# hinike/cairo

Measured on AMD Instinct MI355X. Metric: encoded Mpixels/s (p-frame, q=16) at 1/2/4/8 MI355X; bit-exact vs ref, higher is better.
Workload: dtype int16

## Files before the change

### cairo_amd/__init__.py

```python
from __future__ import annotations

import ctypes
import os
from dataclasses import dataclass

import numpy as np

_HERE = os.path.dirname(os.path.abspath(__file__))
LIB_PATH = os.path.join(_HERE, "_lib", "libcairo_amd.so")

BLOCK_DESC = np.dtype(
    [
        ("block_type", "<u4"),
        ("prediction_target", "u1"),
        ("pad", "u1"),
        ("motion_x", "<i2"),
        ("motion_y", "<i2"),
        ("sp_pred", "u1"),
        ("sp_amount", "u1"),
        ("sp_index", "u1"),
        ("q_index", "u1"),
        ("variance", "<i2"),
    ]
)
# ... 362 lines not shown
    feed: np.ndarray | None = None
    feed_bits: int = 0
    feed_status: int = 0


def _view(addr: int, dtype, count: int) -> np.ndarray:
    buf = (ctypes.c_char * (count * np.dtype(dtype).itemsize)).from_address(addr)
    return np.frombuffer(buf, dtype=dtype, count=count)


class Context:

    def __init__(self, width: int, height: int, ring: int = 4, device: int = 0, stages: int = 96):
        self.L = lib()
        self.width, self.height, self.ring, self.device = width, height, ring, device
        self.wa, self.ha = (width + 15) & ~15, (height + 15) & ~15
        self.wmb, self.hmb = self.wa // 16, self.ha // 16
        p = ctypes.c_void_p()
        _ck(self.L.cairo_ctx_create_ex(width, height, ring, device, stages, ctypes.byref(p)), "cairo_ctx_create")
        self.h = p
        self._keep = {}

    def close(self) -> None:
        if self.h:
            self.L.cairo_ctx_destroy(self.h)
            self.h = None

    def __del__(self):
        try:
            self.close()
        except Exception:
            pass

    @property
    def stages(self) -> int:
        return int(self.L.cairo_ctx_stages(self.h))

    def submit(self, rgb, index: int, inter: bool, quality: int, on_device: bool = False,
               fmt: int = FMT_RGB24, pitch: int = 0, src_size=None, crop=None) -> int:
        t = ctypes.c_int()
        if src_size is not None or crop is not None:
            if src_size is None:
                raise ValueError("crop needs src_size")
            s = _source(src_size, crop)
            ptr = _scaled_source_ptr(rgb, on_device, fmt, src_size, pitch)
            _ck(self.L.cairo_ctx_submit_scaled(self.h, ptr, fmt, pitch, ctypes.byref(s), index, int(inter), quality,
                                               ctypes.byref(t)), "cairo_ctx_submit_scaled")
            return t.value
        ptr = rgb if on_device else _host_frame_fmt(rgb, fmt, self.width, self.height, pitch)
        if fmt == FMT_RGB24 and not pitch:
            _ck(
                self.L.cairo_ctx_submit(self.h, ptr, int(on_device), index, int(inter), quality, ctypes.byref(t)),
                "cairo_ctx_submit",
            )
        else:
            _ck(self.L.cairo_ctx_submit_fmt(self.h, ptr, int(on_device), fmt, pitch, index, int(inter), quality,
                                            ctypes.byref(t)), "cairo_ctx_submit_fmt")
        if not on_device:
            self._keep[t.value] = rgb
        return t.value

    def wait(self, ticket: int, copy: bool = True) -> FrameOutputs:
        r = _FrameResult()
        st = self.L.cairo_ctx_wait(self.h, ticket, ctypes.byref(r))
        if st != EVX_SUCCESS:
            raise CairoError("cairo_ctx_wait", st, self.timeout_info() if st == EVX_ERROR_HARDWAREFAIL else None)
        self._keep.pop(ticket, None)
        return self._outputs(r, copy)

    ACCT_FIELDS = ("coder_tasks", "coder_total", "coder_group_wait", "coder_window", "coder_search", "coder_inter",
                   "coder_dequeue", "coder_mbs", "helper_tasks", "helper_total", "helper_wait", "helper_deblock",
                   "helper_search", "helper_catchup", "helper_dequeue", "helper_chunks",
                   "win_bytes", "win_spec_unused_bytes", "zero_mv_bytes", "gran_poll_bytes", "rec_poll_bytes",
                   "win_stages", "searched_tasks", "inter_tasks", "coder_xform", "coder_publish", "coder_drain",
                   "coder_vm0", "coder_records", "coder_prebarrier", "coder_store_tail",
                   "search_eval", "search_barrier", "search_select", "subpel_eval", "subpel_barrier",
                   "subpel_select", "db_inputs", "db_filter", "db_write",
                   "search_passes", "search_mbs_2pass", "search_mbs_3pass", "search_mbs_4pass",
                   "coder_xform_copy", "coder_copy_mbs", "coder_xform_coded", "coder_coded_mbs",
                   "helper_carry", "carry_bytes",
                   "coder_prologue_fresh", "coder_prologue_records", "helper_group_start",
                   "start_older_searched", "start_ref1_searched", "start_older_idle", "start_ref1_idle",
                   "older_searched", "older_idle", "ref1_idle",
                   "flag_set", "fallback_polls", "fallback_full", "lvl2_runs", "idle_groups", "idle_group_time")

    def read_acct(self, reset: bool = False) -> dict:
        w = np.zeros(len(self.ACCT_FIELDS), np.uint64)
        _ck(self.L.cairo_ctx_read_acct(self.h, _ptr(w), len(w), int(reset)), "cairo_ctx_read_acct")
        return {k: int(w[i]) for i, k in enumerate(self.ACCT_FIELDS)}

    def timeout_info(self) -> dict | None:
        w = np.zeros(16, np.int32)
        _ck(self.L.cairo_ctx_timeout_info(self.h, _ptr(w), 16), "cairo_ctx_timeout_info")
        if not w[0]:
            return None
        d = {k: int(w[i]) for i, k in enumerate(TIMEOUT_FIELDS)}
        d["kind"] = WAIT_KINDS.get(d["kind"], str(d["kind"]))
        d["seen"] = (d.pop("seen_hi") & 0xFFFFFFFF) << 32 | (d.pop("seen_lo") & 0xFFFFFFFF)
        return d

    def _outputs(self, r, copy: bool) -> FrameOutputs:
        ny, nc = r.wa * r.ha, (r.wa // 2) * (r.ha // 2)
        mbs = r.wmb * r.hmb
        has_coef = bool(r.coef_y)
        feed = _view(r.feed, np.uint32, (r.feed_bits + 31) // 32) if r.feed_status == FEED_VALID else None
        out = FrameOutputs(
            _view(r.block_table, BLOCK_DESC, mbs),
            _view(r.coef_y, np.int16, ny).reshape(r.ha, r.wa) if has_coef else None,
            _view(r.coef_u, np.int16, nc).reshape(r.ha // 2, r.wa // 2) if has_coef else None,
            _view(r.coef_v, np.int16, nc).reshape(r.ha // 2, r.wa // 2) if has_coef else None,
            feed, int(r.feed_bits), int(r.feed_status),
        )
        if copy:
            cp = lambda a: None if a is None else a.copy()
            out = FrameOutputs(cp(out.table), cp(out.coef_y), cp(out.coef_u), cp(out.coef_v), cp(out.feed),
                               out.feed_bits, out.feed_status)
        return out

    def set_outputs(self, outputs: int) -> None:
        _ck(self.L.cairo_ctx_set_outputs(self.h, outputs), "cairo_ctx_set_outputs")

    def fetch_coef(self, ticket: int):
        r = _FrameResult()
        _ck(self.L.cairo_ctx_fetch_coef(self.h, ticket, ctypes.byref(r)), "cairo_ctx_fetch_coef")
        ny, nc = self.wa * self.ha, (self.wa // 2) * (self.ha // 2)
        return (_view(r.coef_y, np.int16, ny).reshape(self.ha, self.wa).copy(),
                _view(r.coef_u, np.int16, nc).reshape(self.ha // 2, self.wa // 2).copy(),
                _view(r.coef_v, np.int16, nc).reshape(self.ha // 2, self.wa // 2).copy())

    def set_metrics(self, sse: bool = True, ssim: bool = True, keep_recon: bool = False, flags: int | None = None) -> None:
        if flags is None:
            flags = (METRIC_SSE if sse else 0) | (METRIC_SSIM if ssim else 0) | (KEEP_RECON if keep_recon else 0)
        _ck(self.L.cairo_ctx_set_metrics(self.h, flags), "cairo_ctx_set_metrics")

    def set_input_color(self, range: int, matrix: int) -> None:
        _ck(self.L.cairo_ctx_set_input_color(self.h, range, matrix), "cairo_ctx_set_input_color")

    def set_output_color(self, range: int, matrix: int) -> None:
        _ck(self.L.cairo_ctx_set_output_color(self.h, range, matrix), "cairo_ctx_set_output_color")

    def frame_metrics(self, ticket: int) -> dict:
        m = _FrameMetrics()
        _ck(self.L.cairo_ctx_frame_metrics(self.h, ticket, ctypes.byref(m)), "cairo_ctx_frame_metrics")
        return _metrics_dict(m)

    def fetch_recon_planes(self, ticket: int):
        y = np.empty((self.ha, self.wa), np.int16)
        u = np.empty((self.ha // 2, self.wa // 2), np.int16)
        v = np.empty_like(u)
        _ck(self.L.cairo_ctx_fetch_recon_planes(self.h, ticket, _ptr(y), _ptr(u), _ptr(v)),
            "cairo_ctx_fetch_recon_planes")
        return y, u, v

    def fetch_recon(self, ticket: int, fmt: int, pitch: int = 0, out: np.ndarray | None = None) -> np.ndarray:
        nb, _ = frame_layout(fmt, self.width, self.height, pitch)
        if out is None:
            out = np.zeros(nb, np.uint8)
        elif not isinstance(out, np.ndarray) or out.dtype != np.uint8 or out.nbytes != nb or \
                not out.flags["C_CONTIGUOUS"]:
            raise ValueError(f"out must be a C-contiguous uint8 array of {nb} bytes")
        _ck(self.L.cairo_ctx_fetch_recon(self.h, ticket, fmt, pitch, _ptr(out)), "cairo_ctx_fetch_recon")
        return out

    def release(self, ticket: int) -> None:
        _ck(self.L.cairo_ctx_release(self.h, ticket), "cairo_ctx_release")

    def encode_frame(self, rgb, index: int, inter: bool, quality: int, on_device: bool = False,
# ... 513 lines not shown
```

### cairo_amd/csrc/kernels.h

```cpp
#pragma once

#include <hip/hip_runtime.h>
#include <stddef.h>
#include <stdint.h>

#include "evx_defs.h"

namespace cairo {

struct PlaneSet {
  int16_t* y;
  int16_t* u;
  int16_t* v;
};

__host__ __device__ inline PlaneSet ring_slot(int16_t* base, size_t slot_elems, int wa, int ha,
                                              int k) {
  PlaneSet p;
  p.y = base + (size_t)k * slot_elems;
  p.u = p.y + (size_t)wa * ha;
  p.v = p.u + (size_t)(wa / 2) * (ha / 2);
  return p;
}

constexpr int kGranulesPerMB = 192;
constexpr int kGranuleStride = 193;

__host__ __device__ inline uint32_t pack_inter_desc(const BlockDesc& d) {
  return (d.block_type & 7u) | ((uint32_t)(d.prediction_target & 3) << 3) | ((uint32_t)(d.sp_pred & 1) << 5) |
         ((uint32_t)(d.sp_amount & 1) << 6) | ((uint32_t)(d.sp_index & 15) << 7) |
         (((uint32_t)d.motion_x & 0x7Fu) << 11) | (((uint32_t)d.motion_y & 0x7Fu) << 18);
}
__host__ __device__ inline BlockDesc unpack_inter_desc(uint32_t w) {
  BlockDesc d;
  d.block_type = w & 7u;
  d.prediction_target = (uint8_t)((w >> 3) & 3);
  d.pad = 0;
  d.sp_pred = (uint8_t)((w >> 5) & 1);
  d.sp_amount = (uint8_t)((w >> 6) & 1);
  d.sp_index = (uint8_t)((w >> 7) & 15);
  d.motion_x = (int16_t)((int32_t)(w << 14) >> 25);
  d.motion_y = (int16_t)((int32_t)(w << 7) >> 25);
  d.q_index = 0;
  d.variance = 0;
  return d;
}

constexpr int kStampPhases = 12;
constexpr int kDbStamps = 256;
constexpr int kIStamps = 12;
__host__ __device__ inline size_t stamp_frame_words(int wmb, int hmb) {
  return (size_t)wmb * hmb * kStampPhases + (size_t)hmb * kDbStamps;
}

struct TimeoutInfo {
  static constexpr int kKind = 0;
  static constexpr int kEpoch = 1;
  static constexpr int kIndex = 2;
  static constexpr int kRow = 3;
  static constexpr int kMember = 4;
  static constexpr int kNeed = 5;
  static constexpr int kOn = 6;
  static constexpr int kSeenLo = 7;
  static constexpr int kSeenHi = 8;
  static constexpr int kClaim = 9;
  static constexpr int kWords = 16;
};
enum TimeoutKind : int32_t {
  kWaitRecords = 1,
  kWaitGranule = 2,
  kWaitPrevProgress = 3,
  kWaitRowAbove = 4,
  kWaitBatch = 5,
  kWaitInjected = 6,
  kWaitHostMark = 9,
};

#ifndef CAIRO_ACCT
#define CAIRO_ACCT 0
#endif
constexpr int kAcctShards = 64, kAcctWords = 66;
struct Acct {
  static constexpr int kCoderTasks = 0, kCoderTotal = 1, kCoderGroupWait = 2, kCoderWindow = 3, kCoderSearch = 4,
                       kCoderInter = 5, kCoderDequeue = 6, kCoderMBs = 7;
  static constexpr int kHelperTasks = 8, kHelperTotal = 9, kHelperWait = 10, kHelperDeblock = 11, kHelperSearch = 12,
                       kHelperCatchup = 13, kHelperDequeue = 14, kHelperChunks = 15;
  static constexpr int kWinBytes = 16, kWinSpecUnused = 17, kZeroMvBytes = 18, kGranPollBytes = 19,
                       kRecPollBytes = 20, kWinStages = 21, kSearchedTasks = 22, kInterTasks = 23;
  static constexpr int kCoderXform = 24, kCoderPublish = 25, kCoderDrain = 26;
  static constexpr int kCoderVm0 = 27, kCoderRecords = 28, kCoderPreBarrier = 29;
  static constexpr int kCoderStoreTail = 30;
  static constexpr int kSrchEval = 31, kSrchBarrier = 32, kSrchSelect = 33, kSubEval = 34, kSubBarrier = 35,
                       kSubSelect = 36;
  static constexpr int kDbInputs = 37, kDbFilter = 38, kDbWrite = 39;
  static constexpr int kSrchPasses = 40, kSrchPasses2 = 41, kSrchPasses3 = 42, kSrchPasses4 = 43;
  static constexpr int kCoderXformCopy = 44, kCoderCopyMBs = 45, kCoderXformCoded = 46, kCoderCodedMBs = 47;
  static constexpr int kHelperCarry = 48, kCarryBytes = 49;
  static constexpr int kCoderProFresh = 50, kCoderProRecords = 51, kHelperGroupStart = 52;
  static constexpr int kStartOlderSearched = 53, kStartRef1Searched = 54, kStartOlderIdle = 55, kStartRef1Idle = 56,
                       kOlderSearched = 57, kOlderIdle = 58, kRef1Idle = 59;
  static constexpr int kFlagSet = 60, kFallbackPolls = 61, kFallbackFull = 62, kLvl2Runs = 63;
  static constexpr int kIdleGroups = 64, kIdleGroupTime = 65;
};

#ifndef CAIRO_MAX_BATCH
#define CAIRO_MAX_BATCH 48
#endif
constexpr int kMaxBatch = CAIRO_MAX_BATCH;
constexpr int kMaxGroup = 16;
constexpr int kMaxPush = kMaxRing;

struct FrameDesc {
  const uint8_t* rgb;
  const uint8_t* host_rgb;
  int index;
  int inter;
  int quality;
  uint32_t epoch;
  int slot;
  int decode;
  PlaneSet recon[kMaxRing];
  PlaneSet stale;
  PlaneSet coef;
  PlaneSet push[kMaxPush];
  int npush;
  PlaneSet coef_prev;
  uint64_t* progress;
  const uint64_t* prev_progress;
  const uint64_t* prev2_progress;
  int sys;
  int member;
  const BlockDesc* host_table;
  const int16_t* host_coef;
};

struct alignas(64) FrameArgs {
  int wa, ha;
  int wmb, hmb;
  uint32_t epoch;
  int nrec;
  BlockDesc* inter_desc;
  PlaneSet in;
  uint64_t* granules;
  PlaneSet stale;
  int ring;
  int pad1;
  int32_t* inter_done;
  int ng;
  int sys;
  int nref;
  int inter;
  uint64_t* acct;
  PlaneSet recon[kMaxRing];
  BlockDesc* table;
  int quality;
  int decode;
  int index;
  int member;
  int32_t* err;
  PlaneSet coef;
  PlaneSet coef_prev;
  uint64_t* progress;
  int db_shift;
  int npush;
  const uint64_t* prev_progress;
  const uint64_t* prev2_progress;
  int32_t* sticky;
  uint64_t* istamps;
  const uint8_t* rgb;
  int inject;
  int w, h;
  int pad0;
  uint64_t* stamps;
  PlaneSet push[kMaxPush];
};
struct ViewLayout {
  static constexpr size_t kCoderStart = 0, kStale = 64, kGroup = 96, kPredict = 128, kPublish = 256, kHelper = 320,
                          kPush = 384, kSize = 512;
};
static_assert(offsetof(FrameArgs, wa) == ViewLayout::kCoderStart && offsetof(FrameArgs, ha) == 4 &&
                  offsetof(FrameArgs, wmb) == 8 && offsetof(FrameArgs, hmb) == 12 && offsetof(FrameArgs, epoch) == 16 && offsetof(FrameArgs, nrec) == 20 &&
                  offsetof(FrameArgs, inter_desc) == 24 && offsetof(FrameArgs, in) == 32 &&
                  offsetof(FrameArgs, granules) == 56,
              "FrameArgs block 0: the coder's macroblock start");
static_assert(offsetof(FrameArgs, stale) == ViewLayout::kStale && offsetof(FrameArgs, ring) == 88 &&
// ... 117 lines not shown
```

### cairo_amd/csrc/kernels.hip

```cpp
#include "kernels.h"

namespace cairo {

typedef const __attribute__((address_space(4))) FrameArgs FA;
#define RECON_AT(a, k)                                                                   \
  ((k) == 1 ? planes((a).recon[1]) : (k) == 2 ? planes((a).recon[2]) : (k) == 3 ? planes((a).recon[3]) \
                                                                              : planes((a).recon[0]))
__host__ __device__ inline PlaneSet planes(const __attribute__((address_space(4))) PlaneSet& p) {
  PlaneSet r;
  r.y = p.y;
  r.u = p.u;
  r.v = p.v;
  return r;
}


__constant__ int16_t kLut8[64] = {
    128, 128,  128,  128,  128,  128,  128,  128,
    126, 106,  71,   25,   -25,  -71,  -106, -126,
    118, 49,   -49,  -118, -118, -49,  49,   118,
    106, -25,  -126, -71,  71,   126,  25,   -106,
    91,  -91,  -91,  91,   91,   -91,  -91,  91,
    71,  -126, 25,   106,  -106, -25,  126,  -71,
    49,  -118, 118,  -49,  -49,  118,  -118, 49,
// ... 368 lines not shown
  int16_t u[kWinC * kWinCP];
  int16_t v[kWinC * kWinCP];
};

__device__ __forceinline__ uint4 bias4(uint4 v) {
  v.x ^= 0x80008000u, v.y ^= 0x80008000u, v.z ^= 0x80008000u, v.w ^= 0x80008000u;
  return v;
}

#ifndef CAIRO_ATTR_SKIP
#define CAIRO_ATTR_SKIP 0
#endif
#if CAIRO_ATTR_SKIP && !defined(CAIRO_TOOLS_BUILD)
#error "CAIRO_ATTR_SKIP produces wrong output: tools builds only (define CAIRO_TOOLS_BUILD)"
#endif

typedef __attribute__((address_space(3))) void lds_void;
__device__ __forceinline__ void dma_window(Window& w, const PlaneSet& p, int wa, int ha, int ox, int oy, int r0,
                                           int r1, int c0, int c1) {
  const int wave = threadIdx.x >> 6, lane = threadIdx.x & 63;
  if (CAIRO_ATTR_SKIP & 1) return;
  constexpr int kLC = kWinLP / 8, kCC = kWinCP / 8;
  static_assert(kWinLP % 8 == 0 && kWinCP % 8 == 0, "16-byte chunked pitches");
  const int k0 = r0 * kLC, k1 = r1 * kLC;
  for (int kb = k0 + 64 * wave; kb < k1; kb += 256) {
    const int k = kb + lane, r = k / kLC, cc = k - r * kLC, c = cc << 3;
    const int gy = oy + r, gx = ox + c;
    if (k < k1 && cc < (kWinLW >> 3) && c >= c0 && c < c1 && gy >= 0 && gy < ha && gx >= 0 && gx < wa)
      __builtin_amdgcn_global_load_lds((const void*)&p.y[(size_t)gy * wa + gx], (lds_void*)&w.y[kb << 3], 16, 0, 0);
  }
  const int cr0 = r0 >> 1, cr1 = r1 >> 1, ck0 = cr0 * kCC, ck1 = cr1 * kCC;
  const int ni = (ck1 - ck0 + 63) >> 6;
  const int cw = wa >> 1, ch = ha >> 1, cox = ox >> 1, coy = oy >> 1;
  for (int i = wave; i < 2 * ni; i += 4) {
    const int pl = i >= ni, kb = ck0 + ((i - (pl ? ni : 0)) << 6);
    const int k = kb + lane, r = k / kCC, cc = k - r * kCC, c = cc << 3;
    const int gy = coy + r, gx = cox + c;
    if (k < ck1 && cc < 8 && 2 * c >= c0 && 2 * c < c1 && gy >= 0 && gy < ch && gx >= 0 && gx < cw)
      __builtin_amdgcn_global_load_lds((const void*)&pick(p, 1 + pl)[(size_t)gy * cw + gx],
                                       (lds_void*)&(pl ? w.v : w.u)[kb << 3], 16, 0, 0);
  }
}
__device__ __forceinline__ void bias_window(Window& w, int r0, int r1, int c0, int c1) {
  const int wave = threadIdx.x >> 6, lane = threadIdx.x & 63;
  {
    const int k0 = c0 >> 3, k1 = c1 >> 3;
    const int rr = lane >> 4, kk = lane & 15;
    if (kk >= k0 && kk < k1)
      for (int r = r0 + 4 * wave + rr; r < r1; r += 16) {
        uint4* q = (uint4*)&w.y[r * kWinLP + 8 * kk];
        *q = bias4(*q);
      }
    const int cr0 = r0 >> 1, cr1 = r1 >> 1, ck0 = c0 >> 4, ck1 = c1 >> 4;
    const int crr = lane >> 3, ckk = lane & 7;
    if (ckk >= ck0 && ckk < ck1)
      for (int k = 8 * wave + crr; k < 2 * (cr1 - cr0); k += 32) {
        const int pl = k >= cr1 - cr0, r = cr0 + k - (pl ? cr1 - cr0 : 0);
        uint4* q = (uint4*)&(pl ? w.v : w.u)[r * kWinCP + 8 * ckk];
        *q = bias4(*q);
      }
  }
}
__device__ __forceinline__ void load_window_dma(Window& w, const PlaneSet& p, int wa, int ha, int ox, int oy, int r0,
                                                int r1, int c0, int c1) {
  dma_window(w, p, wa, ha, ox, oy, r0, r1, c0, c1);
  asm volatile("s_waitcnt vmcnt(0)" ::: "memory");
  __syncthreads();
  bias_window(w, r0, r1, c0, c1);
}

__device__ __forceinline__ void acct_window(uint64_t* acct, int r0, int r1, int c0, int c1) {
  acct_add(acct, Acct::kWinBytes, (uint64_t)(r1 - r0) * (c1 - c0) * 3);
  acct_add(acct, Acct::kWinStages, 1);
}
__device__ __forceinline__ void stage_window(Window& w, const PlaneSet& p, int wa, int ha, int ox, int oy, int r0,
                                             int r1, int c0, int c1) {
  load_window_dma(w, p, wa, ha, ox, oy, r0, r1, c0, c1);
}

struct Px6 {
  int y0, y1, y2, y3, u, v;
};

__device__ __forceinline__ Px6 px_from_window_b(const Window& w, int wx, int wy) {
  int l = lane_id();
  const uint16_t* py = (const uint16_t*)&w.y[(wy + (l >> 2)) * kWinLP + wx + (l & 3) * 4];
  int cwx = wx >> 1, cwy = wy >> 1;
  Px6 r;
  r.y0 = py[0];
  r.y1 = py[1];
  r.y2 = py[2];
  r.y3 = py[3];
  r.u = ((const uint16_t*)w.u)[(cwy + (l >> 3)) * kWinCP + cwx + (l & 7)];
  r.v = ((const uint16_t*)w.v)[(cwy + (l >> 3)) * kWinCP + cwx + (l & 7)];
  return r;
}

__device__ __forceinline__ Px6 px_from_planes(const PlaneSet& p, int wa, int x, int y) {
  int l = lane_id();
  const int16_t* py = &p.y[(size_t)(y + (l >> 2)) * wa + x + (l & 3) * 4];
  int cw = wa >> 1;
  Px6 r;
  r.y0 = py[0];
  r.y1 = py[1];
  r.y2 = py[2];
  r.y3 = py[3];
  r.u = p.u[(size_t)((y >> 1) + (l >> 3)) * cw + (x >> 1) + (l & 7)];
  r.v = p.v[(size_t)((y >> 1) + (l >> 3)) * cw + (x >> 1) + (l & 7)];
  return r;
}

__device__ __forceinline__ int lerp_px(int a, int b, int quarter) {
  return quarter ? (int16_t)(round_out(3 * a + b, 2) / 4) : (int16_t)(round_out(a + b, 1) / 2);
}
__device__ __forceinline__ uint32_t lerp_half_bb(uint32_t a, uint32_t b) {
  const uint32_t t = a + b;
  return (t + ((t >> 16) & 1)) >> 1;
}
__device__ __forceinline__ uint32_t lerp_quarter_bb3(uint32_t a3, uint32_t b) {
  const uint32_t t = a3 + b;
  return (t + 1 + ((t >> 17) & 1)) >> 2;
}
__device__ __forceinline__ uint32_t lerp_quarter_bb(uint32_t a, uint32_t b) { return lerp_quarter_bb3(3 * a, b); }
__device__ __forceinline__ uint32_t absdiff_b(uint32_t x, uint32_t y) {
  return __builtin_amdgcn_sad_u16(x, y, 0);
}

__device__ __forceinline__ void inter_cand_row(const Window& w, int wx, int wy, int i, const SrcRow& s, int thr,
                                               int& sad, int& mad) {
  const int sh = (wx & 1) * 2;
  const uint32_t* row = (const uint32_t*)&w.y[(wy + i) * kWinLP] + (wx >> 1);
  uint32_t d[9];
#pragma unroll
  for (int k = 0; k < 9; k++) d[k] = row[k];
  uint32_t sm = 0;
#pragma unroll
  for (int k = 0; k < 8; k++) sm = __builtin_amdgcn_sad_u16(s.y[k], __builtin_amdgcn_alignbyte(d[k + 1], d[k], sh), sm);
  sad = row16_sum((int)sm);
  mad = kMadFar;
  if (__ballot(mad_needed(sad, thr))) {
    u16x2 m1 = {0, 0}, m2 = {0, 0};
    uint32_t dummy = 0;
#pragma unroll
    for (int k = 0; k < 8; k++) pk_diff(s.y[k], __builtin_amdgcn_alignbyte(d[k + 1], d[k], sh), dummy, m1, m2);
    const int cr = (wy >> 1) + (i >> 1), cc = (wx >> 1) + (i & 1) * 4, shc = (cc & 1) * 2;
    const uint32_t* ru = (const uint32_t*)&w.u[cr * kWinCP] + (cc >> 1);
    const uint32_t* rv = (const uint32_t*)&w.v[cr * kWinCP] + (cc >> 1);
    const uint32_t u0 = ru[0], u1 = ru[1], u2 = ru[2], v0 = rv[0], v1 = rv[1], v2 = rv[2];
    pk_diff(s.u[0], __builtin_amdgcn_alignbyte(u1, u0, shc), dummy, m1, m2);
    pk_diff(s.u[1], __builtin_amdgcn_alignbyte(u2, u1, shc), dummy, m1, m2);
    pk_diff(s.v[0], __builtin_amdgcn_alignbyte(v1, v0, shc), dummy, m1, m2);
    pk_diff(s.v[1], __builtin_amdgcn_alignbyte(v2, v1, shc), dummy, m1, m2);
    const u16x2 m = __builtin_elementwise_max(m1, m2);
    mad = row16_max(max((int)m.x, (int)m.y));
  }
}

__device__ __forceinline__ SrcRow load_src_rows(const PlaneSet& in, int wa, int px, int py, int i) {
  SrcRow s;
  const uint4* ry = (const uint4*)(in.y + (size_t)(py + i) * wa + px);
  const uint4 r0 = ry[0], r1 = ry[1];
  s.y[0] = r0.x, s.y[1] = r0.y, s.y[2] = r0.z, s.y[3] = r0.w;
  s.y[4] = r1.x, s.y[5] = r1.y, s.y[6] = r1.z, s.y[7] = r1.w;
  const size_t co = (size_t)((py >> 1) + (i >> 1)) * (wa >> 1) + (px >> 1) + (i & 1) * 4;
  const uint2 u2 = *(const uint2*)(in.u + co), v2 = *(const uint2*)(in.v + co);
  s.u[0] = u2.x, s.u[1] = u2.y, s.v[0] = v2.x, s.v[1] = v2.y;
#pragma unroll
  for (int k = 0; k < 8; k++) s.y[k] ^= 0x80008000u;
#pragma unroll
  for (int k = 0; k < 2; k++) s.u[k] ^= 0x80008000u, s.v[k] ^= 0x80008000u;
  return s;
}

__device__ __forceinline__ void sad_mad(const Px6& s, const Px6& c, int& sad, int& mad) {
  int d0 = abs(s.y0 - c.y0), d1 = abs(s.y1 - c.y1), d2 = abs(s.y2 - c.y2), d3 = abs(s.y3 - c.y3);
  int du = abs(s.u - c.u), dv = abs(s.v - c.v);
  sad = wave_sum(d0 + d1 + d2 + d3);
  mad = wave_max(max(max(max(d0, d1), max(d2, d3)), max(du, dv)));
}

struct Sel {
  int bx, by, sad, mad, ssd, sp_idx, sp_amt, sp_en;
};

__device__ __forceinline__ void accept_int(Sel& s, int cx, int cy, int sad, int mad, int px, int py,
                                           int thr) {
  int ssd = (cx - px) * (cx - px) + (cy - py) * (cy - py);
  bool acc = (s.mad < thr) ? (mad < s.mad || (mad == s.mad && ssd < s.ssd))
                           : (sad < s.sad || (sad == s.sad && ssd < s.ssd && sad < kSadGate) ||
                              mad < thr);
  if (acc) {
    s.bx = cx;
    s.by = cy;
    s.sad = sad;
    s.ssd = ssd;
    s.mad = mad;
  }
}
__device__ __forceinline__ void accept_sub(Sel& s, int idx, int quarter, int sad, int mad,
                                           int thr) {
  bool acc = (s.mad < thr) ? (mad < s.mad) : ((sad < s.sad && sad < kSadGate) || mad < thr);
  if (acc) {
    s.sp_en = 1;
    s.sp_amt = quarter;
    s.sp_idx = idx;
    s.sad = sad;
    s.mad = mad;
  }
}



__device__ __forceinline__ uint32_t row0_min(uint32_t v) {
  v = min(v, (uint32_t)__builtin_amdgcn_mov_dpp((int)v, 0x128, 0xF, 0xF, false));
  v = min(v, (uint32_t)__builtin_amdgcn_mov_dpp((int)v, 0x124, 0xF, 0xF, false));
  v = min(v, (uint32_t)__builtin_amdgcn_mov_dpp((int)v, 0x122, 0xF, 0xF, false));
  v = min(v, (uint32_t)__builtin_amdgcn_mov_dpp((int)v, 0x121, 0xF, 0xF, false));
  return (uint32_t)__builtin_amdgcn_readlane((int)v, 0);
}

__device__ __forceinline__ uint32_t key_copy(int mad, int ssd, int idx) {
  return ((uint32_t)min(mad, 65535) << 16) | ((uint32_t)min(ssd, 4095) << 4) | (uint32_t)idx;
}
__device__ __forceinline__ uint32_t key_sad(int sad, int ssd, int idx) {
  if (sad < kSadGate)
    return ((uint32_t)sad << 18) | ((uint32_t)min(ssd, 16383) << 4) | (uint32_t)idx;
  return 0x80000000u | ((uint32_t)min(sad, (1 << 27) - 1) << 4) | (uint32_t)idx;
}

__device__ __forceinline__ void select_int(Sel& s, bool valid, int cx, int cy, int sad, int mad,
                                           int px, int py, int thr, int lane) {
  const int c = lane & 15;
  const bool live = lane < 16 && valid;
  const int ssd = (cx - px) * (cx - px) + (cy - py) * (cy - py);
  const uint32_t fm = (uint32_t)__ballot(live && mad < thr);
  int w = -1;
  if (s.mad < thr || fm) {
    const int f = s.mad < thr ? -1 : (int)__builtin_ctz(fm);
// ... 238 lines not shown
  s.v[0] = m[160 + co] ^ 0x80008000u, s.v[1] = m[160 + co + 1] ^ 0x80008000u;
  return s;
}

__device__ __forceinline__ void zero_mv_older(FA& a, int r, int g, InterLds& L) {
  const int wave = threadIdx.x >> 6, x = 4 * g + wave;
  acct_add(a.acct, Acct::kZeroMvBytes, 768ull * (a.nref - 1) * (uint64_t)min(4, a.wmb - 4 * g));
  if (x < a.wmb) {
    const int px = x * kMB, py = r * kMB;
    const int thr = (a.quality >> 2) + 1;
    const Px6 src = src_px_lds(L, wave);
    Px6 ref[kMaxRing - 1];
#pragma unroll
    for (int off = 2; off < kMaxRing; off++)
      if (off <= a.nref) ref[off - 1] = px_from_planes(RECON_AT(a, off), a.wa, px, py);
#pragma unroll
    for (int off = 2; off < kMaxRing; off++) {
      if (off > a.nref) break;
      int sad, mad;
      sad_mad(src, ref[off - 1], sad, mad);
      if ((threadIdx.x & 63) == 0) {
        L.zsad[off][wave] = sad, L.zmad[off][wave] = mad;
        L.zneed[off][wave] = mad >= thr && !(CAIRO_ATTR_SKIP & 8);
      }
    }
  } else if ((threadIdx.x & 63) == 0) {
#pragma unroll
    for (int off = 2; off < kMaxRing; off++) L.zneed[off][wave] = 0;
  }
  __syncthreads();
}

#ifndef CAIRO_CODER_CARRY
#define CAIRO_CODER_CARRY 0
#endif

typedef uint32_t u32x4 __attribute__((ext_vector_type(4)));
typedef __attribute__((address_space(1))) u32x4 gbl_u32x4;
typedef uint32_t u32x2 __attribute__((ext_vector_type(2)));
typedef u32x2 u32x2_u __attribute__((aligned(2)));
__device__ __forceinline__ void store16_through(bool sys, int16_t* p, u32x4 v) {
  if (sys)
    asm volatile("global_store_dwordx4 %0, %1, off sc0 sc1" ::"v"(p), "v"(v) : "memory");
  else
    asm volatile("global_store_dwordx4 %0, %1, off sc1" ::"v"(p), "v"(v) : "memory");
}

__device__ __forceinline__ bool carry_wanted(FA& a) {
  return !CAIRO_CODER_CARRY && planes(a.coef).y != planes(a.coef_prev).y;
}
__device__ __forceinline__ ptrdiff_t carry_chunk(FA& a, int r, int g, int& pl) {
  const int t = threadIdx.x;
  int row, x, col;
  if (t < 128) {
    pl = 0, row = r * kMB + (t >> 3), x = 4 * g + ((t & 7) >> 1), col = 4 * g * kMB + 8 * (t & 7);
  } else {
    const int k = t - 128;
    pl = 1 + (k >> 5), row = r * (kMB / 2) + ((k & 31) >> 2), x = 4 * g + (k & 3), col = x * (kMB / 2);
  }
  if (t >= 192 || x >= a.wmb) return -1;
  return (ptrdiff_t)((size_t)row * (pl ? a.wa >> 1 : a.wa) + col);
}
__device__ __forceinline__ u32x4 carry_load(FA& a, int pl, ptrdiff_t off) {
  return *(const gbl_u32x4*)(pick(planes(a.coef_prev), pl) + off);
}
__device__ __forceinline__ void carry_store(FA& a, int pl, ptrdiff_t off, u32x4 v) {
  store16_through(a.sys, pick(planes(a.coef), pl) + off, v);
}

template <bool kRef1>
__device__ __forceinline__ bool inter_task(FA& a0, int r, int g, int off, InterLds& L, DbLds& D, DbState& st,
                                           int* flag, uint64_t* is, bool carried = false) {
  FA& a = *opaque_view(&a0);
  ASM_MARK("group_start begin");
  const uint64_t tg0 = acct_now();
  const int wave = uni(threadIdx.x >> 6);
  const int x = 4 * g + wave;
  const bool valid = x < a.wmb;
  const int px = x * kMB, py = r * kMB, mb = r * a.wmb + x;
  const int mbs = a.wmb * a.hmb;
  const int thr = (a.quality >> 2) + 1;
  const PlaneSet ref = RECON_AT(a, off);
  Sel s;
  Px6 src;
  s.bx = px;
  s.by = py;
  s.ssd = INT32_MAX;
  s.sp_idx = s.sp_amt = s.sp_en = 0;
  s.sad = s.mad = 0;
  SrcRow srow;
  const int ox = 4 * g * kMB - 32, oy = py - 32;
  const uint64_t* pp = kRef1 ? a.prev_progress : a.prev2_progress;
  const uint64_t want = tagged(a.epoch - (kRef1 ? 1 : 2), inter_need_cols(a, g, 2));
  const bool wf = uni(L.wfull[kRef1 ? 0 : 1]) != 0 || !pp;
  bool need = false;
  bool any, full = wf;
  if (kRef1) {
    int cpl = 0;
    const ptrdiff_t coff = carried ? carry_chunk(a, r, g, cpl) : -1;
    const uint64_t tc0 = acct_now();
    u32x4 cv = {0, 0, 0, 0};
    if (coff >= 0) cv = carry_load(a, cpl, coff);
    u32x2 zy = {0, 0};
    int zu = 0, zv = 0;
    if (valid) {
      const int l = lane_id();
      const size_t co = (size_t)((py >> 1) + (l >> 3)) * (a.wa >> 1) + (px >> 1) + (l & 7);
      zy = *(const u32x2_u*)&ref.y[(size_t)(py + (l >> 2)) * a.wa + px + (l & 3) * 4];
      zu = ref.u[co], zv = ref.v[co];
    }
    const bool poll = threadIdx.x == 0 && !wf;
    uint64_t w3 = 0, w2 = 0;
    if (poll) {
      w3 = progress_peer(a.sys, pp + min(r + 3, a.hmb - 1));
      w2 = progress_peer(a.sys, pp + min(r + 2, a.hmb - 1));
    }
    asm volatile("" : "+v"(cv), "+v"(zy), "+v"(zu), "+v"(zv), "+v"(w3), "+v"(w2));
    if (coff >= 0) carry_store(a, cpl, coff, cv);
    Px6 zref;
    zref.y0 = (int16_t)zy.x, zref.y1 = (int16_t)(zy.x >> 16), zref.y2 = (int16_t)zy.y, zref.y3 = (int16_t)(zy.y >> 16);
    zref.u = zu, zref.v = zv;
    if (carried) {
      acct_add(a.acct, Acct::kHelperCarry, acct_now() - tc0);
      acct_add(a.acct, Acct::kCarryBytes, 768ull * (uint64_t)min(4, a.wmb - 4 * g));
    }
    if (valid) {
      src = src_px_lds(L, wave);
      srow = src_rows_lds(L, wave, threadIdx.x & 15);
      sad_mad(src, zref, s.sad, s.mad);
    }
    need = valid && s.mad >= thr && !(CAIRO_ATTR_SKIP & 8);
    if ((threadIdx.x & 63) == 0) L.need[wave] = need;
    if (threadIdx.x == 0) {
      int f = wf;
      if (poll) {
        f = (w3 >= want) & (w2 >= want);
        if (f) {
          acquire_fence(a.sys);
          asm volatile("s_waitcnt vmcnt(0)" ::: "memory");
        }
        acct_start(a.acct, Acct::kFallbackFull, f);
      }
      L.full = f;
    }
    __syncthreads();
    any = uni(L.need[0] | L.need[1] | L.need[2] | L.need[3]) != 0;
    full = uni(L.full) != 0;
    if (is) is[3] = __builtin_amdgcn_s_memrealtime();
  } else {
    any = uni(L.zneed[off][0] | L.zneed[off][1] | L.zneed[off][2] | L.zneed[off][3]) != 0;
    if (valid) {
      src = src_px_lds(L, wave);
      srow = src_rows_lds(L, wave, threadIdx.x & 15);
      s.sad = L.zsad[off][wave], s.mad = L.zmad[off][wave];
      need = L.zneed[off][wave] != 0;
    }
    if (any && !wf) {
      if (threadIdx.x == 0) {
        const uint64_t w3 = progress_peer(a.sys, pp + min(r + 3, a.hmb - 1));
        const uint64_t w2 = progress_peer(a.sys, pp + min(r + 2, a.hmb - 1));
        const int f = (w3 >= want) & (w2 >= want);
        if (f) {
          acquire_fence(a.sys);
          asm volatile("s_waitcnt vmcnt(0)" ::: "memory");
        }
        acct_start(a.acct, Acct::kFallbackFull, f);
        L.full = f;
      }
      __syncthreads();
      full = uni(L.full) != 0;
    }
  }
  acct_add(a.acct, Acct::kInterTasks, 1);
  acct_add(a.acct, Acct::kZeroMvBytes, (kRef1 ? 768ull : 0ull) * (uint64_t)min(4, a.wmb - 4 * g));
  if (kRef1 || any) {
    acct_start(a.acct, Acct::kFlagSet, wf);
    acct_start(a.acct, Acct::kFallbackPolls, !wf);
  }
  if (any) {
    acct_add(a.acct, Acct::kSearchedTasks, 1);
    acct_window(a.acct, 0, full ? kWinL : kLvl1Rows, 0, full ? kWinLW : kLvl1Cols);
    acct_add(a.acct, Acct::kHelperGroupStart, acct_now() - tg0);
    acct_start(a.acct, kRef1 ? Acct::kStartRef1Searched : Acct::kStartOlderSearched, acct_now() - tg0);
    acct_start(a.acct, Acct::kOlderSearched, kRef1 ? 0 : 1);
    ASM_MARK("group_start end");
    stage_window(L.win, ref, a.wa, a.ha, ox, oy, 0, full ? kWinL : kLvl1Rows, 0, full ? kWinLW : kLvl1Cols);
    __syncthreads();
    if (is && off == 1) is[4] = __builtin_amdgcn_s_memrealtime();
    bool lvl2c = full, lvl2r = full;
    bool lvl2_open = true;
    for (int si = 0; si < 6; si++) {
      const int step = si < 5 ? kRadius >> si : 1;
      if (!lvl2r && lvl2_open) {
        const int rem = si < 5 ? 2 * step : 1;
        const int want = need ? (s.by + step - oy > kLvl1Rows - kMB) * 2 + (!lvl2c && s.bx + step - ox > kLvl1Cols - kMB)
                              : 0;
        const int may = need && (s.by + rem - oy > kLvl1Rows - kMB || (!lvl2c && s.bx + rem - ox > kLvl1Cols - kMB));
        if ((threadIdx.x & 63) == 0) L.lvl2[si][wave] = want | (may << 2);
        __syncthreads();
        const int m4 = L.lvl2[si][0] | L.lvl2[si][1] | L.lvl2[si][2] | L.lvl2[si][3];
        const int m = m4 & 3;
        lvl2_open = (m4 >> 2) != 0;
        if (m) {
          if (is) is[5] = __builtin_amdgcn_s_memrealtime();
          acct_start(a.acct, Acct::kLvl2Runs, 1);
          helper_wait<false>(a, off == 1 ? 1 : 2, r, min(r + ((m & 2) ? 3 : 2), a.hmb - 1), inter_need_cols(a, g, 2),
                             D, st, flag);
          if (m & 2) stage_window(L.win, ref, a.wa, a.ha, ox, oy, kLvl1Rows, kWinL, 0, kWinLW);
          if (!lvl2c) stage_window(L.win, ref, a.wa, a.ha, ox, oy, 0, kLvl1Rows, kLvl1Cols, kWinLW);
          if (m & 2) acct_window(a.acct, kLvl1Rows, kWinL, 0, kWinLW);
          if (!lvl2c) acct_window(a.acct, 0, kLvl1Rows, kLvl1Cols, kWinLW);
          __syncthreads();
          if (is) is[6] = __builtin_amdgcn_s_memrealtime(), is[7] += (m & 2) ? 0x10000 : 1;
          lvl2c = true;
          lvl2r = (m & 2) != 0;
        }
      }
      if (is && off == 1 && (si == 1 || si == 5)) is[si == 1 ? 8 : 9] = __builtin_amdgcn_s_memrealtime();
      if (!need) continue;
      if (si < 5) {
        const int bx = s.bx, by = s.by;
        const int lane = threadIdx.x & 63, gi = lane & 15, grp = lane >> 4;
        const int my_pass = gi < 4 ? 0 : 1, my_grp = gi < 4 ? gi : gi - 5;
        int sadv = s.sad, madv = s.mad;
#pragma unroll
        for (int pass = 0; pass < 2; pass++) {
          const int c = 4 * pass + grp + (pass > 0);
          const int cx = bx + (c % 3 - 1) * step, cy = by + (c / 3 - 1) * step;
          const bool ok = in_frame(cx, cy, a.wa, a.ha);
          int sad, mad;
          inter_cand_row(L.win, (ok ? cx : bx) - ox, (ok ? cy : by) - oy, gi, srow, thr, sad, mad);
          const int from = (16 * (my_grp & 3)) << 2;
          const int vs = __builtin_amdgcn_ds_bpermute(from, sad), vm = __builtin_amdgcn_ds_bpermute(from, mad);
          if (my_pass == pass && gi != 4) sadv = vs, madv = vm;
        }
        {
          const int cx = bx + (gi % 3 - 1) * step, cy = by + (gi / 3 - 1) * step;
          select_int(s, gi < 9 && in_frame(cx, cy, a.wa, a.ha), cx, cy, sadv, madv, px, py, thr, lane);
        }
      } else {
        const Px6 best = px_from_window_b(L.win, s.bx - ox, s.by - oy);
        s.sp_idx = s.sp_amt = s.sp_en = 0;
        const int bx = s.bx, by = s.by;
        const uint32_t sb0 = src.y0 + 0x8000, sb1 = src.y1 + 0x8000, sb2 = src.y2 + 0x8000, sb3 = src.y3 + 0x8000,
                       sbu = src.u + 0x8000, sbv = src.v + 0x8000;
        const uint32_t b30 = 3 * best.y0, b31 = 3 * best.y1, b32 = 3 * best.y2, b33 = 3 * best.y3, b3u = 3 * best.u,
                       b3v = 3 * best.v;
#pragma unroll
        for (int n = 0; n < 8; n++) {
          const int k9 = n < 4 ? n : n + 1, i = k9 % 3 - 1, j = k9 / 3 - 1, tx = bx + i, ty = by + j;
          const bool ok = in_frame(tx, ty, a.wa, a.ha);
          if (!ok) continue;
          const Px6 nb = px_from_window_b(L.win, tx - ox, ty - oy);
          const int idx = frac_index(i, j);
#pragma unroll
          for (int q = 0; q < 2; q++) {
            const uint32_t d0 = absdiff_b(sb0, q ? lerp_quarter_bb3(b30, nb.y0) : lerp_half_bb(best.y0, nb.y0)),
                           d1 = absdiff_b(sb1, q ? lerp_quarter_bb3(b31, nb.y1) : lerp_half_bb(best.y1, nb.y1)),
                           d2 = absdiff_b(sb2, q ? lerp_quarter_bb3(b32, nb.y2) : lerp_half_bb(best.y2, nb.y2)),
                           d3 = absdiff_b(sb3, q ? lerp_quarter_bb3(b33, nb.y3) : lerp_half_bb(best.y3, nb.y3)),
                           du = absdiff_b(sbu, q ? lerp_quarter_bb3(b3u, nb.u) : lerp_half_bb(best.u, nb.u)),
                           dv = absdiff_b(sbv, q ? lerp_quarter_bb3(b3v, nb.v) : lerp_half_bb(best.v, nb.v));
            const int lsum = (int)(d0 + d1 + d2 + d3);
            const int lmax = (int)max(max(max(d0, d1), d2), max(max(d3, du), dv));
            const bool copy = s.mad < thr;
            const bool mad_lt = __ballot(lmax >= (copy ? s.mad : thr)) == 0;
            int sad = 0;
            bool acc;
            if (copy) {
              acc = mad_lt;
            } else {
              sad = wave_sum(lsum);
              acc = (sad < s.sad && sad < kSadGate) || mad_lt;
            }
            if (acc) {
              s.sp_en = 1;
              s.sp_amt = q;
              s.sp_idx = idx;
              s.sad = copy ? wave_sum(lsum) : sad;
              s.mad = wave_max(lmax);
            }
          }
        }
      }
    }
  } else if (carried) {
    asm volatile("s_waitcnt vmcnt(0)" ::: "memory");
    __syncthreads();
  }
  if (!any) {
    acct_start(a.acct, kRef1 ? Acct::kStartRef1Idle : Acct::kStartOlderIdle, acct_now() - tg0);
    acct_start(a.acct, kRef1 ? Acct::kRef1Idle : Acct::kOlderIdle, 1);
  }
  if (is && off == 1) is[10] = __builtin_amdgcn_s_memrealtime();
  if (valid && (threadIdx.x & 63) == 0) {
    const BlockDesc d = make_desc(s, px, py, thr, false, off);
    uint64_t* rec = (uint64_t*)&a.inter_desc[(off - 1) * mbs + mb];
    const uint64_t tag = (uint64_t)a.epoch << 32;
    gran_st(rec, tag | pack_inter_desc(d));
    gran_st(rec + 1, tag | (uint32_t)s.sad);
  }
  if (kRef1 || any) asm volatile("s_waitcnt lgkmcnt(0)\n\ts_barrier" ::: "memory");
  return any;
}


constexpr int kMBElems = 384;
typedef short int8v __attribute__((ext_vector_type(8)));

__device__ __forceinline__ void elem_coords(int e, int x, int y, int& plane, int& ex, int& ey) {
  int b = e >> 6, r = (e >> 3) & 7, c = e & 7;
  if (b < 4) {
    plane = 0;
    ex = x + (b & 1) * 8 + c;
    ey = y + (b >> 1) * 8 + r;
  } else {
    plane = b - 3;
    ex = (x >> 1) + c;
    ey = (y >> 1) + r;
  }
}


__device__ __forceinline__ int8v load_row8(const int16_t* p) {
  return *(const int8v*)p;
}

__device__ __forceinline__ int fdct_lane(int16_t* sa, int16_t* sb, int lane, int16_t x) {
  const int r8 = lane >> 3, c8 = lane & 7;
  sa[lane] = x;
  __builtin_amdgcn_wave_barrier();
  {
    const int8v row = load_row8(&sa[r8 * 8]), lut = load_row8(&sLut8[c8 * 8]);
    int t = 0;
#pragma unroll
    for (int k = 0; k < 8; k++) t += row[k] * lut[k];
    t = c8 == 0 ? (t * 45) / 128 : t / 2;
    sb[c8 * 8 + r8] = (int16_t)rdiv(t, 128);
  }
  __builtin_amdgcn_wave_barrier();
  const int8v col = load_row8(&sb[c8 * 8]), lut = load_row8(&sLut8[r8 * 8]);
  int t = 0;
#pragma unroll
  for (int k = 0; k < 8; k++) t += col[k] * lut[k];
  t = r8 == 0 ? (t * 45) / 128 : t / 2;
  return (int16_t)rdiv(t, 128);
}

__device__ __forceinline__ int idct_lane(int16_t* sa, int16_t* sb, int lane, int16_t d) {
  const int r8 = lane >> 3, c8 = lane & 7;
  sa[c8 * 8 + r8] = d;
  __builtin_amdgcn_wave_barrier();
  {
    const int8v col = load_row8(&sa[c8 * 8]), lut = load_row8(&sLut8T[r8 * 8]);
    int t = ((col[0] * lut[0]) * 45) / 128;
#pragma unroll
    for (int k = 1; k < 8; k++) t += (col[k] * lut[k]) / 2;
    sb[r8 * 8 + c8] = (int16_t)rdiv(t, 128);
  }
  __builtin_amdgcn_wave_barrier();
  const int8v row = load_row8(&sb[r8 * 8]), lut = load_row8(&sLut8T[c8 * 8]);
  int t = ((row[0] * lut[0]) * 45) / 128;
#pragma unroll
  for (int k = 1; k < 8; k++) t += (row[k] * lut[k]) / 2;
  return rdiv(t, 128);
// ... 1439 lines not shown
```

Before: 7449.

## Parallelize sub-pel refinement across lane groups with row-based packed interpolation

Replaces the serial per-candidate sub-pel loop with a row-oriented evaluation. Four 16-lane groups each handle a neighbour candidate and compute half- and quarter-pel SAD/MAD together using packed u16 lerps and alignbyte. Results are gathered with ds_bpermute and a new select_sub picks the winner, cutting serial wave reductions from 16 per MB to two rounds. Chroma MAD is evaluated only when needed. The risk is bit-exactness of the new lerp/selection order against the previous sequential acceptance logic, and select_sub is not shown here. Also adds accounting counters for the helper sub-pel phase.

```diff
diff --git a/cairo_amd/__init__.py b/cairo_amd/__init__.py
--- a/cairo_amd/__init__.py
+++ b/cairo_amd/__init__.py
@@ -468,7 +468,8 @@
                    "coder_prologue_fresh", "coder_prologue_records", "helper_group_start",
                    "start_older_searched", "start_ref1_searched", "start_older_idle", "start_ref1_idle",
                    "older_searched", "older_idle", "ref1_idle",
-                   "flag_set", "fallback_polls", "fallback_full", "lvl2_runs", "idle_groups", "idle_group_time")
+                   "flag_set", "fallback_polls", "fallback_full", "lvl2_runs", "idle_groups", "idle_group_time",
+                   "helper_subpel", "helper_subpel_runs")
 
     def read_acct(self, reset: bool = False) -> dict:
         w = np.zeros(len(self.ACCT_FIELDS), np.uint64)
diff --git a/cairo_amd/csrc/kernels.h b/cairo_amd/csrc/kernels.h
--- a/cairo_amd/csrc/kernels.h
+++ b/cairo_amd/csrc/kernels.h
@@ -79,7 +79,7 @@
 #ifndef CAIRO_ACCT
 #define CAIRO_ACCT 0
 #endif
-constexpr int kAcctShards = 64, kAcctWords = 66;
+constexpr int kAcctShards = 64, kAcctWords = 68;
 struct Acct {
   static constexpr int kCoderTasks = 0, kCoderTotal = 1, kCoderGroupWait = 2, kCoderWindow = 3, kCoderSearch = 4,
                        kCoderInter = 5, kCoderDequeue = 6, kCoderMBs = 7;
@@ -101,6 +101,7 @@
                        kOlderSearched = 57, kOlderIdle = 58, kRef1Idle = 59;
   static constexpr int kFlagSet = 60, kFallbackPolls = 61, kFallbackFull = 62, kLvl2Runs = 63;
   static constexpr int kIdleGroups = 64, kIdleGroupTime = 65;
+  static constexpr int kHelperSubpel = 66, kHelperSubpelRuns = 67;
 };
 
 #ifndef CAIRO_MAX_BATCH
diff --git a/cairo_amd/csrc/kernels.hip b/cairo_amd/csrc/kernels.hip
--- a/cairo_amd/csrc/kernels.hip
+++ b/cairo_amd/csrc/kernels.hip
@@ -474,20 +474,6 @@
   int y0, y1, y2, y3, u, v;
 };
 
-__device__ __forceinline__ Px6 px_from_window_b(const Window& w, int wx, int wy) {
-  int l = lane_id();
-  const uint16_t* py = (const uint16_t*)&w.y[(wy + (l >> 2)) * kWinLP + wx + (l & 3) * 4];
-  int cwx = wx >> 1, cwy = wy >> 1;
-  Px6 r;
-  r.y0 = py[0];
-  r.y1 = py[1];
-  r.y2 = py[2];
-  r.y3 = py[3];
-  r.u = ((const uint16_t*)w.u)[(cwy + (l >> 3)) * kWinCP + cwx + (l & 7)];
-  r.v = ((const uint16_t*)w.v)[(cwy + (l >> 3)) * kWinCP + cwx + (l & 7)];
-  return r;
-}
-
 __device__ __forceinline__ Px6 px_from_planes(const PlaneSet& p, int wa, int x, int y) {
   int l = lane_id();
   const int16_t* py = &p.y[(size_t)(y + (l >> 2)) * wa + x + (l & 3) * 4];
@@ -514,9 +500,6 @@
   return (t + 1 + ((t >> 17) & 1)) >> 2;
 }
 __device__ __forceinline__ uint32_t lerp_quarter_bb(uint32_t a, uint32_t b) { return lerp_quarter_bb3(3 * a, b); }
-__device__ __forceinline__ uint32_t absdiff_b(uint32_t x, uint32_t y) {
-  return __builtin_amdgcn_sad_u16(x, y, 0);
-}
 
 __device__ __forceinline__ void inter_cand_row(const Window& w, int wx, int wy, int i, const SrcRow& s, int thr,
                                                int& sad, int& mad) {
@@ -546,6 +529,70 @@
     const u16x2 m = __builtin_elementwise_max(m1, m2);
     mad = row16_max(max((int)m.x, (int)m.y));
   }
+}
+
+__device__ __forceinline__ void lerp_pair_hq(uint32_t a, uint32_t b, uint32_t& lh, uint32_t& lq) {
+  const uint32_t x = a ^ b;
+  const u16x2 fl = as_u16x2(a & b) + (as_u16x2(x) >> 1);
+  const uint32_t f = __builtin_bit_cast(uint32_t, fl);
+  lh = __builtin_bit_cast(uint32_t, fl + as_u16x2(__builtin_bit_cast(uint32_t, fl >> 15) & x));
+  const uint32_t y = a ^ f;
+  const u16x2 v = as_u16x2(a & f) + (as_u16x2(y) >> 1);
+  lq = __builtin_bit_cast(uint32_t, v + as_u16x2(y & (x | __builtin_bit_cast(uint32_t, v >> 15)) & 0x00010001u));
+}
+__device__ __forceinline__ u16x2 pk_absdiff(uint32_t a, uint32_t b) {
+  return __builtin_elementwise_sub_sat(as_u16x2(a), as_u16x2(b)) |
+         __builtin_elementwise_sub_sat(as_u16x2(b), as_u16x2(a));
+}
+
+static_assert(kWinLW - kMB + 18 <= kWinLP, "a sub-pel row read stays inside the luma pitch");
+static_assert((kWinLW - kMB) / 2 + 4 + 6 <= kWinCP, "... and the chroma pitch");
+__device__ __forceinline__ void inter_subpel_rows(const Window& w, int bwx, int bwy, int nwx, int nwy, int i,
+                                                  const SrcRow& s, int thr, int& sadh, int& madh, int& sadq,
+                                                  int& madq) {
+  const int sha = (bwx & 1) * 2, shb = (nwx & 1) * 2;
+  const uint32_t* ra = (const uint32_t*)&w.y[(bwy + i) * kWinLP] + (bwx >> 1);
+  const uint32_t* rb = (const uint32_t*)&w.y[(nwy + i) * kWinLP] + (nwx >> 1);
+  uint32_t smh = 0, smq = 0;
+  u16x2 mh = {0, 0}, mq = {0, 0};
+#pragma unroll
+  for (int h = 0; h < 2; h++) {
+    uint32_t da[5], db[5];
+    if (h) asm volatile("" ::: "memory");
+#pragma unroll
+    for (int k = 0; k < 5; k++) da[k] = ra[4 * h + k], db[k] = rb[4 * h + k];
+#pragma unroll
+    for (int k = 0; k < 4; k++) {
+      uint32_t lh, lq;
+      lerp_pair_hq(__builtin_amdgcn_alignbyte(da[k + 1], da[k], sha), __builtin_amdgcn_alignbyte(db[k + 1], db[k], shb),
+                   lh, lq);
+      const u16x2 dh = pk_absdiff(s.y[4 * h + k], lh), dq = pk_absdiff(s.y[4 * h + k], lq);
+      smh = __builtin_amdgcn_sad_u16(__builtin_bit_cast(uint32_t, dh), 0u, smh);
+      smq = __builtin_amdgcn_sad_u16(__builtin_bit_cast(uint32_t, dq), 0u, smq);
+      mh = __builtin_elementwise_max(mh, dh), mq = __builtin_elementwise_max(mq, dq);
+    }
+  }
+  sadh = row16_sum((int)smh), sadq = row16_sum((int)smq);
+  madh = madq = kMadFar;
+  if (!__ballot(mad_needed(min(sadh, sadq), thr))) return;
+  const int cra = (bwy >> 1) + (i >> 1), crb = (nwy >> 1) + (i >> 1);
+  const int xa = (bwx >> 1) + (i & 1) * 4, xb = (nwx >> 1) + (i & 1) * 4;
+  const int sca = (xa & 1) * 2, scb = (xb & 1) * 2;
+#pragma unroll
+  for (int pl = 0; pl < 2; pl++) {
+    const int16_t* t = pl ? w.v : w.u;
+    const uint32_t* pa = (const uint32_t*)&t[cra * kWinCP] + (xa >> 1);
+    const uint32_t* pb = (const uint32_t*)&t[crb * kWinCP] + (xb >> 1);
+    const uint32_t a0 = pa[0], a1 = pa[1], a2 = pa[2], b0 = pb[0], b1 = pb[1], b2 = pb[2];
+    const uint32_t* sp = pl ? s.v : s.u;
+    uint32_t lh, lq;
+    lerp_pair_hq(__builtin_amdgcn_alignbyte(a1, a0, sca), __builtin_amdgcn_alignbyte(b1, b0, scb), lh, lq);
+    mh = __builtin_elementwise_max(mh, pk_absdiff(sp[0], lh)), mq = __builtin_elementwise_max(mq, pk_absdiff(sp[0], lq));
+    lerp_pair_hq(__builtin_amdgcn_alignbyte(a2, a1, sca), __builtin_amdgcn_alignbyte(b2, b1, scb), lh, lq);
+    mh = __builtin_elementwise_max(mh, pk_absdiff(sp[1], lh)), mq = __builtin_elementwise_max(mq, pk_absdiff(sp[1], lq));
+  }
+  madh = row16_max(max((int)mh.x, (int)mh.y));
+  madq = row16_max(max((int)mq.x, (int)mq.y));
 }
 
 __device__ __forceinline__ SrcRow load_src_rows(const PlaneSet& in, int wa, int px, int py, int i) {
@@ -950,7 +997,6 @@
   const int thr = (a.quality >> 2) + 1;
   const PlaneSet ref = RECON_AT(a, off);
   Sel s;
-  Px6 src;
   s.bx = px;
   s.by = py;
   s.ssd = INT32_MAX;
@@ -993,9 +1039,8 @@
       acct_add(a.acct, Acct::kCarryBytes, 768ull * (uint64_t)min(4, a.wmb - 4 * g));
     }
     if (valid) {
-      src = src_px_lds(L, wave);
       srow = src_rows_lds(L, wave, threadIdx.x & 15);
-      sad_mad(src, zref, s.sad, s.mad);
+      sad_mad(src_px_lds(L, wave), zref, s.sad, s.mad);
     }
     need = valid && s.mad >= thr && !(CAIRO_ATTR_SKIP & 8);
     if ((threadIdx.x & 63) == 0) L.need[wave] = need;
@@ -1018,7 +1063,6 @@
   } else {
     any = uni(L.zneed[off][0] | L.zneed[off][1] | L.zneed[off][2] | L.zneed[off][3]) != 0;
     if (valid) {
-      src = src_px_lds(L, wave);
       srow = src_rows_lds(L, wave, threadIdx.x & 15);
       s.sad = L.zsad[off][wave], s.mad = L.zmad[off][wave];
       need = L.zneed[off][wave] != 0;
@@ -1107,48 +1151,30 @@
           select_int(s, gi < 9 && in_frame(cx, cy, a.wa, a.ha), cx, cy, sadv, madv, px, py, thr, lane);
         }
       } else {
-        const Px6 best = px_from_window_b(L.win, s.bx - ox, s.by - oy);
+        if (CAIRO_ATTR_SKIP & 128) continue;
+        const uint64_t tsp = acct_now();
         s.sp_idx = s.sp_amt = s.sp_en = 0;
         const int bx = s.bx, by = s.by;
-        const uint32_t sb0 = src.y0 + 0x8000, sb1 = src.y1 + 0x8000, sb2 = src.y2 + 0x8000, sb3 = src.y3 + 0x8000,
-                       sbu = src.u + 0x8000, sbv = src.v + 0x8000;
-        const uint32_t b30 = 3 * best.y0, b31 = 3 * best.y1, b32 = 3 * best.y2, b33 = 3 * best.y3, b3u = 3 * best.u,
-                       b3v = 3 * best.v;
-#pragma unroll
-        for (int n = 0; n < 8; n++) {
-          const int k9 = n < 4 ? n : n + 1, i = k9 % 3 - 1, j = k9 / 3 - 1, tx = bx + i, ty = by + j;
+        const int lane = threadIdx.x & 63, gi = lane & 15, grp = lane >> 4;
+        const int from = (16 * ((gi >> 1) & 3) + (gi & 1)) << 2;
+        int sadv = 0, madv = 0;
+#pragma unroll 1
+        for (int rd = 0; rd < 2; rd++) {
+          const int n = 4 * rd + grp, k9 = n < 4 ? n : n + 1;
+          const int tx = bx + k9 % 3 - 1, ty = by + k9 / 3 - 1;
           const bool ok = in_frame(tx, ty, a.wa, a.ha);
-          if (!ok) continue;
-          const Px6 nb = px_from_window_b(L.win, tx - ox, ty - oy);
-          const int idx = frac_index(i, j);
-#pragma unroll
-          for (int q = 0; q < 2; q++) {
-            const uint32_t d0 = absdiff_b(sb0, q ? lerp_quarter_bb3(b30, nb.y0) : lerp_half_bb(best.y0, nb.y0)),
-                           d1 = absdiff_b(sb1, q ? lerp_quarter_bb3(b31, nb.y1) : lerp_half_bb(best.y1, nb.y1)),
-                           d2 = absdiff_b(sb2, q ? lerp_quarter_bb3(b32, nb.y2) : lerp_half_bb(best.y2, nb.y2)),
-                           d3 = absdiff_b(sb3, q ? lerp_quarter_bb3(b33, nb.y3) : lerp_half_bb(best.y3, nb.y3)),
-                           du = absdiff_b(sbu, q ? lerp_quarter_bb3(b3u, nb.u) : lerp_half_bb(best.u, nb.u)),
-                           dv = absdiff_b(sbv, q ? lerp_quarter_bb3(b3v, nb.v) : lerp_half_bb(best.v, nb.v));
-            const int lsum = (int)(d0 + d1 + d2 + d3);
-            const int lmax = (int)max(max(max(d0, d1), d2), max(max(d3, du), dv));
-            const bool copy = s.mad < thr;
-            const bool mad_lt = __ballot(lmax >= (copy ? s.mad : thr)) == 0;
-            int sad = 0;
-            bool acc;
-            if (copy) {
-              acc = mad_lt;
-            } else {
-              sad = wave_sum(lsum);
-              acc = (sad < s.sad && sad < kSadGate) || mad_lt;
-            }
-            if (acc) {
-              s.sp_en = 1;
-              s.sp_amt = q;
-              s.sp_idx = idx;
-              s.sad = copy ? wave_sum(lsum) : sad;
-              s.mad = wave_max(lmax);
-            }
-          }
+          int sadh, madh, sadq, madq;
+          inter_subpel_rows(L.win, bx - ox, by - oy, (ok ? tx : bx) - ox, (ok ? ty : by) - oy, gi, srow, thr, sadh,
+                            madh, sadq, madq);
+          const int vs = __builtin_amdgcn_ds_bpermute(from, ok ? ((gi & 1) ? sadq : sadh) : -1),
+                    vm = __builtin_amdgcn_ds_bpermute(from, (gi & 1) ? madq : madh);
+          if ((gi >> 3) == rd) sadv = vs, madv = vm;
+        }
+        select_sub(s, sadv >= 0, sadv, madv, thr, lane);
+        if (CAIRO_ACCT) {
+          const uint64_t tse = uni((int)s.sp_idx) == -99999 ? 0 : acct_now();
+          acct_add(a.acct, Acct::kHelperSubpel, tse - tsp);
+          acct_add(a.acct, Acct::kHelperSubpelRuns, 1);
         }
       }
     }
```

Result: no change. 7523, median of 6 (+1.0%).
